# everpeace/kube-throttler

Measured on AMD Instinct MI355X. Metric: pod_throttle_decisions_per_sec, higher is better.
Workload: dtype int64; 1 GPU; configs[2]: 1M pods x 1k Throttle+ClusterThrottle, D=8; pods_total=1000000, pods_per_gpu=1000000, throttles=1000, dims=8, labels_per_pod=8, namespaces=64, step=reconcile(aggregate+allreduce+finalize,apply)+check(all pods), streams=one, kernel_variant=indexed, parallelism=pods row-sharded x1, throttles replicated, exchange=none

## Files before the change

### kube_throttler_amd/csrc/kt_kernels_check.hip

```cpp
#include <type_traits>

#include "kt_scan.h"

#ifdef KT_PROFILE_PHASES
__device__ unsigned long long kt_prof_check[16];
extern "C" int kt_debug_prof_check(unsigned long long* out16, int reset) {
  if (hipMemcpyFromSymbol(out16, HIP_SYMBOL(kt_prof_check), 16 * 8) != hipSuccess) return -1;
  if (reset) { unsigned long long z[16] = {0}; (void)hipMemcpyToSymbol(HIP_SYMBOL(kt_prof_check), z, 16 * 8); }
  return 0;
}
#define KT_PROF_T(var) const unsigned long long var = __builtin_amdgcn_s_memtime()
#define KT_PROF_ADD(slot, dt) prof_acc[slot] += (dt)
#else
#define KT_PROF_T(var)
#define KT_PROF_ADD(slot, dt)
#endif

namespace kt {


constexpr uint32_t kListCap = 128;
template <int DT>
struct alignas(16) WordVerdict {
  uint64_t seg_lo, seg_hi;
  uint64_t tight;
  uint64_t exc;
  uint64_t act;
  uint64_t ins;
  uint64_t act_nib[DT / 4][16];
};
constexpr uint32_t kTiAdj = 0x00100000u, kTiTight = 0x10000000u;
constexpr int kTiShActive = 16, kTiShIdle = 22;

template <int DT, bool WORDWISE, class TI, class WV>
__device__ __forceinline__ void build_term_verdicts(uint32_t tt, uint32_t c, const u32x2* g_rflags, TI* tinfo, WV* wv) {
  const bool real = (tt & kTermReal) != 0;
  const uint32_t t = tt & kTermRowMask;
  const u32x2 rf = real ? g_rflags[t] : u32x2{0u, 0u};
  u32x2 ti = {0u, 0u};
  if (real) {
    const uint32_t sh_act = (rf.x & kRecExceedsByCount) ? 4u : 24u;
    const uint32_t sh_idle = (rf.x & kRecExceedsByCount) ? 4u : (rf.x & kRecActiveByCount) ? 24u : (rf.x & kRecInsufficientByCount) ? 44u : 0u;
    ti.x = t | ((tt & kTermAdj) ? kTiAdj : 0u);
    ti.y = (rf.y & 0xFFFFu) | sh_act << kTiShActive | sh_idle << kTiShIdle | ((rf.x & kRecTight) ? kTiTight : 0u);
  }
  tinfo[c] = ti;
  if (WORDWISE) {
    const uint32_t ln = c & 63u;
    const uint32_t tp = (uint32_t)__shfl_up((int)tt, 1), tn = (uint32_t)__shfl_down((int)tt, 1);
    const bool adj = (tt & kTermAdj) != 0;
    const bool same_prev = ln > 0u && adj && (tp & kTermReal) && (tp & kTermAdj) && (tp & kTermRowMask) == t;
    const bool same_next = ln < 63u && adj && (tn & kTermReal) && (tn & kTermAdj) && (tn & kTermRowMask) == t;
    const bool xc = (rf.x & kRecExceedsByCount) != 0;
    const uint64_t m_lo = __ballot(real && !same_prev), m_hi = __ballot(real && !same_next);
    const uint64_t m_tight = __ballot(real && (rf.x & kRecTight) != 0), m_exc = __ballot(real && xc);
    const uint64_t m_act = __ballot(real && (rf.x & kRecActiveByCount) != 0), m_ins = __ballot(real && (rf.x & kRecInsufficientByCount) != 0);
    WV* wvp = wv + (c >> 6);
    const uint64_t mine = ln == 0u ? m_lo : ln == 1u ? m_hi : ln == 2u ? m_tight : ln == 3u ? m_exc : ln == 4u ? m_act : m_ins;
    const uint32_t eq = ln >> 4, ev = ln & 15u;
    uint64_t tab = m_act;
#pragma unroll
    for (int d = 0; d < DT; ++d) {
      const uint64_t m = __ballot(real && ((rf.y >> d) & 1u) != 0);
      tab |= ((uint32_t)(d >> 2) == eq && ((ev >> (d & 3)) & 1u)) ? m : 0ull;
    }
    typedef decltype(&wvp->seg_lo) u64p;
    if (ln < 6u) ((u64p)wvp)[ln] = mine;
    if (ln < 4u * (uint32_t)DT) ((u64p)wvp)[6u + ln] = tab;
  }
}
template <int DT>
__host__ __device__ constexpr uint32_t verdict_image_word_bytes() { return 64u * 8u; }

template <int DT>
__global__ __launch_bounds__(256) void kt_build_verdict_images(const unsigned char* blob, const BmChunk* chunks, const void* recs, int T,
                                                               uint32_t total_words, unsigned char* out) {
  const BmChunk ch = chunks[blockIdx.y];
  const uint32_t w = blockIdx.x * 4u + (threadIdx.x >> 6);
  if (w >= ch.n_words) return;
  const u32x2* g_rflags = (const u32x2*)rec_flags<DT>((void*)recs, T);
  const uint32_t* term_t = (const uint32_t*)(blob + ch.img_off + ch.off_term_t);
  const uint32_t c_local = w * 64u + (threadIdx.x & 63u);
  const uint32_t c_glob = (ch.w0 + w) * 64u + (threadIdx.x & 63u);
  build_term_verdicts<DT, true>(term_t[c_local], c_glob, g_rflags, (u32x2*)out, (WordVerdict<DT>*)(out + (size_t)total_words * 64u * 8u));
}
size_t verdict_images_bytes(uint32_t total_words, int D) {
  return (size_t)total_words * (64u * 8u + (D <= 8 ? sizeof(WordVerdict<8>) : sizeof(WordVerdict<16>))) + 64;
}
void launch_build_verdict_images(const IndexDev& ix, uint32_t total_words, const void* recs, int T, int D, void* out, hipStream_t s) {
  if (!ix.n_chunks || !ix.bm_max_words) return;
  const dim3 g_((ix.bm_max_words + 3u) / 4u, ix.n_chunks), b_(256);
  if (dt_bucket_ix(D) <= 8) hipLaunchKernelGGL(kt_build_verdict_images<8>, g_, b_, 0, s, ix.bm_blob, ix.bm_chunks, recs, T, total_words, (unsigned char*)out);
  else hipLaunchKernelGGL(kt_build_verdict_images<16>, g_, b_, 0, s, ix.bm_blob, ix.bm_chunks, recs, T, total_words, (unsigned char*)out);
}

template <bool CACHED>
struct TileMatchWords {};
template <>
struct TileMatchWords<true> {
  uint64_t mx[kMatchReplay];
};
template <int LA, int NV = 1, bool CACHED = false>
struct TileRec : TileMatchWords<CACHED> {
  uint32_t p;
  uint64_t meta;
  u32x4 raw[LA / 8];
  unsigned long long carried;
  int64_t v[NV];
};

struct BmCheckArgs {
  const uint64_t* meta;
  const uint16_t* latom;
  const int64_t* req;
  const uint32_t* lpair;
  const uint32_t* lkey;
  const int64_t* rows;
  const void* recs;
  uint64_t* summary;
  uint8_t* status;
  const SelProgram* sp;
  const uint8_t* ns_valid;
  const uint32_t* slow_thr;
  int64_t n;
  BmIndexArgs ix;
  uint32_t off_cnt, off_list, off_tinfo, off_wv;
  uint32_t off_next;
  uint32_t n_slow;
  int32_t DS, LS, T;
  uint32_t* ticket;
  uint64_t* host_summary;
  uint32_t has_overflow;
  const uint64_t* v_meta;
  const uint16_t* v_latom;
  uint64_t* carry;
  const uint32_t* wg_range;
  uint32_t n_inline;
  int64_t inline_rows[8];
  const unsigned char* wv_img;
  uint32_t wv_total_words;
  unsigned char* slab;
  uint32_t* slab_tag;
  uint32_t epoch;
  uint32_t off_rank, off_tab;
  uint32_t pk_nw, pk_rec;
  uint32_t pk_dim[8];
  MatchCacheArgs mc;
};

static BmCheckArgs make_bm_check_args(const PodTable& pods, int64_t n, const int64_t* rows, const SelProgram& sp,
                                      const SelProgram* sp_dev, const IndexDev& ix, const void* recs,
                                      uint64_t* summary, uint8_t* status, uint32_t* total, const PackPlan* agg_pk = nullptr) {
  BmCheckArgs a{};
  a.meta = pods.meta, a.latom = pods.latom, a.req = pods.req, a.lpair = pods.lpair, a.lkey = pods.lkey;
  a.n = n, a.rows = rows, a.recs = recs, a.summary = summary, a.status = status;
  a.sp = sp_dev, a.ns_valid = sp.ns_valid, a.slow_thr = ix.slow_thr, a.n_slow = ix.n_slow;
  a.DS = pods.DS, a.LS = pods.LS, a.T = sp.T;
  uint32_t o = 0;
  auto take = [&](uint32_t bytes) { uint32_t r = o; o += (bytes + 15u) & ~15u; return r; };
  a.off_cnt = take(kBlockIx * 8);
  a.off_list = take((kBlockIx / kWave) * kListCap * 4);
  a.off_next = take(16);
  a.off_tinfo = take(ix.bm_max_words * 64u * 8u);
  a.off_wv = take(ix.bm_max_words * (uint32_t)(pods.D <= 8 ? sizeof(WordVerdict<8>) : sizeof(WordVerdict<16>)));
  plan_bitmap_index(ix, a.ix, take);
  if (agg_pk) {
    a.pk_nw = agg_pk->nw, a.pk_rec = agg_pk->rec_bytes;
    for (int d = 0; d < 8; ++d)
      a.pk_dim[d] = (uint32_t)agg_pk->shift[d] | (uint32_t)agg_pk->pos[d] << 8 | (uint32_t)agg_pk->word[d] << 16 | (agg_pk->width[d] ? 1u << 24 : 0u);
    a.off_rank = take(ix.bm_max_words * 64u * 2u);
    a.off_tab = take(ix.bm_max_thr * agg_pk->rec_bytes);
  }
  *total = o;
  return a;
}

int check_sweep_blocks(int64_t n) {
  const int64_t nb = (n + kBlockIx - 1) / kBlockIx;
  return (int)(nb > kCUs ? kCUs : nb < 1 ? 1 : nb);
}
uint32_t check_fixed_lds() { return kBlockIx * 8 + (kBlockIx / kWave) * kListCap * 4 + 64; }
static_assert(sizeof(WordVerdict<16>) == 560 && 64u * 8u + sizeof(WordVerdict<16>) == kCheckWordLds, "kCheckWordLds (kt_index.h) follows WordVerdict");
static_assert(sizeof(WordVerdict<8>) == 304, "WordVerdict<8>");
uint32_t check_word_lds(int D) { return 64u * 8u + (uint32_t)(D <= 8 ? sizeof(WordVerdict<8>) : sizeof(WordVerdict<16>)); }

template <int DT, int LA, bool VETO, int NEED, int WPE, bool FULL, bool SMALL, bool ONE = false, bool AGG = false, bool CACHED = false>
__global__ __launch_bounds__(kBlockIx, WPE) void kt_check_bitmap(const BmCheckArgs a) {
  static_assert(!AGG || (ONE && !FULL && !SMALL && WPE < 8), "the fused sweep is the lean single-chunk form, one workgroup per CU");
  static_assert(!CACHED || (ONE && !FULL && !SMALL && !AGG && WPE >= 8 && !VETO && NEED == 2 && DT == 8), "the cached form is the lean two-per-CU sweep (one instantiation: nothing of the scan's form is left in it)");
  constexpr int kDrainUnroll = WPE >= 8 ? 1 : (DT / 2 > 4 ? 4 : DT / 2);
  constexpr int kDrainFinalUnroll = WPE >= 8 ? 2 : (DT / 2 > 4 ? 4 : DT / 2);
  constexpr bool WORDWISE = !FULL;
  constexpr bool PREFETCH = WPE < 8;
#ifdef KT_PROFILE_PHASES
  unsigned long long prof_acc[8] = {0, 0, 0, 0, 0, 0, 0, 0};
  KT_PROF_T(t_kernel0);
#endif
  KT_LDS unsigned char* lds = (KT_LDS unsigned char*)kt_smem;
  const CheckRec<DT>* recs = (const CheckRec<DT>*)a.recs;
  const u32x2* g_rflags = (const u32x2*)rec_flags<DT>((void*)a.recs, a.T);
  const uint32_t n = (uint32_t)a.n;
  const int DS = a.DS;
  const uint32_t lane = threadIdx.x & (kWave - 1);
  const uint32_t wave = __builtin_amdgcn_readfirstlane(threadIdx.x / kWave);
  lds_u64wp cnt = (lds_u64wp)(lds + a.off_cnt) + wave * kWave;
  lds_u32wp list = (lds_u32wp)(lds + a.off_list) + wave * kListCap;
  KT_LDS u32x2* tinfo = (KT_LDS u32x2*)(lds + a.off_tinfo);
  const uint32_t n_wtiles = (n + kWave - 1) / kWave;
  const uint32_t wstep = gridDim.x * (kBlockIx / kWave);
  const uint32_t n_chunks = ONE ? 1u : a.ix.n_chunks;
  const uint32_t c_lo = SMALL ? blockIdx.x : 0u, c_hi = SMALL ? blockIdx.x + 1u : n_chunks;
  const bool by_ns = !SMALL && !ONE && a.ix.by_ns != 0u;
  uint32_t t_lo = 0, t_hi = n_wtiles, ns_lo = 0, ns_hi = 0, first_ci = 0u, last_ci = n_chunks - 1u;
  uint32_t rec0 = 0, rec_end = n;
  if (by_ns) {
    if (a.wg_range) {
      rec0 = __builtin_amdgcn_readfirstlane(a.wg_range[blockIdx.x]), rec_end = __builtin_amdgcn_readfirstlane(a.wg_range[blockIdx.x + 1u]);
      if (rec0 >= rec_end) return;
      t_lo = 0u, t_hi = (rec_end - rec0 + kWave - 1u) / kWave;
    } else {
      const uint32_t tpb = (n_wtiles + gridDim.x - 1u) / gridDim.x;
      t_lo = min(blockIdx.x * tpb, n_wtiles), t_hi = min(t_lo + tpb, n_wtiles);
      if (t_lo >= t_hi) return;
    }
    ns_lo = (uint32_t)(a.v_meta[(uint64_t)rec0 + (uint64_t)t_lo * kWave] & kMetaNsMask);
    ns_hi = (uint32_t)(a.v_meta[min((uint64_t)rec0 + (uint64_t)t_hi * kWave, (uint64_t)rec_end) - 1u] & kMetaNsMask);
    ns_lo = __builtin_amdgcn_readfirstlane(ns_lo), ns_hi = __builtin_amdgcn_readfirstlane(max(ns_hi, ns_lo));
    relevant_chunk_span(a.ix, ns_lo, ns_hi, first_ci, last_ci);
    last_ci = max(last_ci, first_ci);
  }
  for (uint32_t ci = SMALL ? c_lo : first_ci; ci < (SMALL ? c_hi : last_ci + 1u); ++ci) {
    if (by_ns && ci != first_ci && !chunk_relevant(a.ix, ci, ns_lo, ns_hi)) continue;
    const bool first = ONE || ci == (SMALL ? 0u : first_ci), last = ONE || ci == last_ci;
    const BmChunk ch = a.ix.chunks[ci];
    const uint32_t wt0 = SMALL ? (wave == 0 ? blockIdx.y : n_wtiles) : by_ns ? t_lo + wave : blockIdx.x * (kBlockIx / kWave) + wave;
    const uint32_t wt_step = SMALL ? n_wtiles : by_ns ? (uint32_t)(kBlockIx / kWave) : wstep;
    auto fetch_tile = [&](uint32_t wt) {
      TileRec<LA, AGG ? DT : 1, CACHED> r;
      const uint32_t i = rec0 + wt * kWave + lane;
      const uint32_t ic = min(i, rec_end - 1u);
      r.p = CACHED ? ic : (SMALL && a.n_inline) ? (uint32_t)a.inline_rows[ic & 7u] : a.rows ? (uint32_t)a.rows[ic] : ic;
      r.meta = by_ns ? a.v_meta[ic] : a.meta[r.p];
      if constexpr (CACHED) load_match_words(a.mc, r.p, r.mx);
      else load_atoms<LA>(by_ns ? a.v_latom : a.latom, by_ns ? ic : r.p, r.raw);
      const unsigned long long* carry_w = by_ns ? (const unsigned long long*)a.carry + ic : (const unsigned long long*)a.summary + (by_ns ? r.p : i);
      r.carried = (!SMALL && !first && i < rec_end) ? __hip_atomic_load(carry_w, __ATOMIC_RELAXED, __HIP_MEMORY_SCOPE_AGENT) : 0ull;
      if constexpr (AGG) load_requests<DT>(a.req, DS, (int64_t)r.p, r.v);
      return r;
    };
    TileRec<LA, AGG ? DT : 1, CACHED> cur{};
    KT_PROF_T(t_b0);
    __syncthreads();
    KT_PROF_T(t_b1);
    KT_PROF_ADD(0, t_b1 - t_b0);
    const BmView bm = open_chunk<VETO>(lds, a.ix, ch);
    if (by_ns && threadIdx.x == 0) *(lds_u32wp)(lds + a.off_next) = t_lo;
    const bool from_images = !SMALL && !ONE && !FULL && a.wv_img != nullptr;
    const uint32_t* term_t = (const uint32_t*)(a.ix.blob + ch.img_off + ch.off_term_t);
    uint32_t tt_first = 0u;
    if (!from_images && threadIdx.x < ch.n_words * 64u) tt_first = term_t[threadIdx.x];
    {
      const u32x4* img0 = (const u32x4*)(a.ix.blob + ch.img_off);
      StageSeg segs[4] = {chunk_image_segment(a.ix, ch), StageSeg{0u, img0, 0u}, StageSeg{0u, img0, 0u}, StageSeg{0u, img0, 0u}};
      if constexpr (CACHED)
        segs[0] = StageSeg{a.ix.lds_img + ch.off_nsl_rng, (const u32x4*)(a.ix.blob + ch.img_off + ch.off_nsl_rng), (ch.lds_bytes - ch.off_nsl_rng) / 16u};
      if constexpr (AGG) segs[1] = StageSeg{a.off_rank, (const u32x4*)(a.ix.blob + ch.img_off + ch.off_term_rank), ch.n_words * 8u};
      if (from_images) {
        segs[2] = StageSeg{a.off_tinfo, (const u32x4*)(a.wv_img + (size_t)ch.w0 * verdict_image_word_bytes<DT>()), ch.n_words * (64u * 8u / 16u)};
        if (WORDWISE)
          segs[3] = StageSeg{a.off_wv, (const u32x4*)(a.wv_img + (size_t)a.wv_total_words * 64u * 8u + (size_t)ch.w0 * sizeof(WordVerdict<DT>)),
                             ch.n_words * (uint32_t)(sizeof(WordVerdict<DT>) / 16u)};
      }
      lds_stage_segments<4>(lds, segs);
    }
    if constexpr (AGG) {
      const uint32_t tab_bytes = (ch.n_thr * a.pk_rec + 15u) & ~15u;
      for (uint32_t i = threadIdx.x; i < tab_bytes / 4; i += kBlockIx) ((lds_u32wp)(lds + a.off_tab))[i] = 0u;
    }
    if (from_images) {
    } else {
      for (uint32_t c = threadIdx.x; c < ch.n_words * 64u; c += kBlockIx)
        build_term_verdicts<DT, WORDWISE>(c == threadIdx.x ? tt_first : term_t[c], c, g_rflags, tinfo, (KT_LDS WordVerdict<DT>*)(lds + a.off_wv));
    }
    KT_PROF_T(t_b2);
    __syncthreads();
    KT_PROF_T(t_b3);
    KT_PROF_ADD(1, t_b2 - t_b1);
    KT_PROF_ADD(2, t_b3 - t_b2);
    KT_PROF_ADD(6, 1ull);
    auto next_tile = [&](uint32_t prev) -> uint32_t {
      if (by_ns) {
        uint32_t t = 0u;
        if (lane == 0u) t = lds_add((lds_u32wp)(lds + a.off_next), 1u);
        return __builtin_amdgcn_readfirstlane(t);
      }
      return prev + wt_step;
    };
    uint32_t wt = by_ns ? next_tile(0u) : wt0;
    uint32_t wt_next = 0u;
    for (; wt < t_hi; wt = wt_next) {
      KT_PROF_T(t_f0);
      cur = fetch_tile(wt);
#ifdef KT_PROFILE_PHASES
      __builtin_amdgcn_s_waitcnt(0);
      KT_PROF_T(t_f1);
      KT_PROF_ADD(3, t_f1 - t_f0);
      KT_PROF_ADD(7, 1ull);
#endif
      const uint32_t i = rec0 + wt * kWave + lane;
      const bool in = i < rec_end;
      const uint32_t ic = min(i, rec_end - 1u);
      const uint32_t p = cur.p;
      const uint32_t si = by_ns ? p : i;
      const uint64_t meta = cur.meta;
      u32x4 raw[LA / 8];
#pragma unroll
      for (int q = 0; q < LA / 8; ++q) raw[q] = CACHED ? u32x4{0u, 0u, 0u, 0u} : cur.raw[q];
      unsigned long long* carry_w = by_ns ? (unsigned long long*)a.carry + ic : (unsigned long long*)a.summary + si;
      const unsigned long long carried = cur.carried;
      cnt[lane] = 0ull;
      unsigned long long my = carried & ~3ull;
      const bool on = in && ((meta >> kMetaStateShift) & kPodValid) != 0;
      const uint32_t ns = on ? (uint32_t)(meta & kMetaNsMask) : 0u;
      const uint32_t nz = (uint32_t)(meta >> kMetaNzShift);
      const uint32_t ns_ok_raw = a.ns_valid[ns];
      bool pod_err = (carried & 2ull) != 0;
      uint32_t ro[LA];
      if constexpr (!CACHED) atom_row_offsets<LA>(raw, ro);
      uint32_t n_list = 0;
      uint32_t last_t = 0xFFFFFFFFu;
      bool counted = false;
      uint32_t zero_keys = 0u;
      unsigned long long pw[4] = {0ull, 0ull, 0ull, 0ull};
      if constexpr (AGG) {
        const uint32_t st = (uint32_t)(meta >> kMetaStateShift) & 0xFu;
        counted = in && (st & (kPodValid | kPodSchedMatch | kPodScheduled | kPodFinished)) == (kPodValid | kPodSchedMatch | kPodScheduled);
        const uint32_t present = (uint32_t)(meta >> kMetaPresentShift) & 0xFFFFu;
        zero_keys = present & ~nz & 0xFFFFu;
        pw[0] = 1ull;
        static_assert(!AGG || DT == 8, "pk_dim holds eight dimensions");
#pragma unroll
        for (int d = 0; d < 8; ++d) {
          const uint32_t pd = a.pk_dim[d];
          const uint64_t f = (uint64_t)cur.v[d] >> (pd & 63u);
          const uint64_t piece = (pd >> 24) ? f << ((pd >> 8) & 63u) : 0ull;
          const uint32_t k = (pd >> 16) & 3u;
          pw[0] |= k == 0u ? piece : 0ull, pw[1] |= k == 1u ? piece : 0ull, pw[2] |= k == 2u ? piece : 0ull, pw[3] |= k == 3u ? piece : 0ull;
        }
      }

      auto drain = [&](auto unroll_tag) {
        constexpr int UNROLL = decltype(unroll_tag)::value;
        for (uint32_t base = 0; base < n_list; base += kWave) {
          const uint32_t j = base + lane;
          const bool vv = j < n_list;
          const uint32_t e = list[vv ? j : 0u];
          const uint32_t pl = e >> 20;
          u32x2 ti = {0u, 0u};
          if (WORDWISE) ti = tinfo[e & kTermRowMask];
          const uint32_t t = WORDWISE ? ti.x & kTermRowMask : e & kTermRowMask;
          const uint32_t prow = (uint32_t)__shfl((int)p, (int)pl);
          const uint32_t psi = FULL ? (uint32_t)__shfl((int)si, (int)pl) : 0u;
          const uint32_t pnz = (uint32_t)__shfl((int)nz, (int)pl);
          const CheckRec<DT>* rc = recs + t;
          const kt_i64x2* xr = (const kt_i64x2*)(a.req + (uint64_t)prow * (uint32_t)DS);
          u32x2 fa;
          if (WORDWISE) {
            const uint32_t sh_act = (ti.y >> kTiShActive) & 63u, sh_idle = (ti.y >> kTiShIdle) & 63u;
            fa.x = (sh_act == 4u ? kRecExceedsByCount : 0u) | (sh_idle == 24u ? kRecActiveByCount : 0u) | (sh_idle == 44u ? kRecInsufficientByCount : 0u);
            fa.y = ti.y & 0xFFFFu;
          } else {
            fa = g_rflags[t];
          }
          bool exc = false, ins = false;
#pragma unroll 1
          for (int q0 = 0; q0 < DT / 2; q0 += UNROLL) {
            kt_i64x2 x[UNROLL], th[UNROLL], hd[UNROLL];
#pragma unroll
            for (int u = 0; u < UNROLL; ++u) {
              const int q = q0 + u;
              x[u] = xr[2 * q < DS ? q : 0];
// ... 87 lines not shown
#pragma unroll
        for (int k = 0; k < DT / 4; ++k) r.nib[k] = *(KT_LDS const unsigned long long*)(q + (PREFETCH ? nib_off[k] : nib_offset(k)));
        return r;
      };
      KT_LDS const uint16_t* trank = (KT_LDS const uint16_t*)(lds + a.off_rank);
      KT_LDS unsigned char* tab = lds + a.off_tab;
      const uint32_t pk_rec = AGG ? a.pk_rec : 0u, pk_nw = AGG ? a.pk_nw : 0u;
      auto fold = [&](uint32_t w, uint64_t x) {
        uint64_t xf = counted ? x : 0ull;
        auto add = [&](bool has, uint32_t r) {
          if (has) {
            KT_LDS unsigned char* rp = tab + __umul24(r, pk_rec);
            lds_u64wp tv = (lds_u64wp)rp;
            lds_add64(tv, pw[0]);
            if (pk_nw > 1u) lds_add64(tv + 1, pw[1]);
            if (pk_nw > 2u) lds_add64(tv + 2, pw[2]);
            if (pk_nw > 3u) lds_add64(tv + 3, pw[3]);
            if (zero_keys) (void)__hip_atomic_fetch_or((lds_u32wp)(rp + pk_nw * 8u), zero_keys, __ATOMIC_RELAXED, __HIP_MEMORY_SCOPE_WORKGROUP);
          }
        };
        while (__ballot(xf != 0ull) != 0ull) {
          const bool h1 = xf != 0ull;
          const uint32_t c1 = h1 ? w * 64u + (uint32_t)__ffsll((unsigned long long)xf) - 1u : 0u;
          xf &= xf - 1ull;
          const bool h2 = xf != 0ull;
          const uint32_t c2 = h2 ? w * 64u + (uint32_t)__ffsll((unsigned long long)xf) - 1u : 0u;
          xf &= xf - 1ull;
          const uint32_t r1 = trank[c1] & 0x7FFFu, r2 = trank[c2] & 0x7FFFu;
          add(h1, r1);
          add(h2, r2);
        }
      };
      auto settle = [&](uint32_t w, uint64_t x, const VerdictRegs& q) -> uint64_t {
        if (seg_on) {
          const uint64_t v = x | q.seg.y;
          x = andn_64(x, v - q.seg.x);
        }
        if constexpr (AGG) fold(w, x);
        uint64_t act = q.nib[0];
#pragma unroll
        for (int k = 1; k < DT / 4; ++k) act |= q.nib[k];
        const uint64_t xe = and_not_and_64(x, q.te.x, q.te.y);
        const uint64_t xf = and_not_not_64(x, q.te.x, q.te.y);
        const uint64_t xa = xf & act, xi = and_not_and_64(xf, act, q.ai.y);
        n_exc = (uint32_t)__popc((uint32_t)xe) + ((uint32_t)__popc((uint32_t)(xe >> 32)) + n_exc);
        n_act = (uint32_t)__popc((uint32_t)xa) + ((uint32_t)__popc((uint32_t)(xa >> 32)) + n_act);
        n_ins = (uint32_t)__popc((uint32_t)xi) + ((uint32_t)__popc((uint32_t)(xi >> 32)) + n_ins);
        return x & q.te.x;
      };
      auto confirm_slow = [&](uint32_t c) {
        return term_match_mem(*a.sp, bm.term_g[c], a.lpair + (uint64_t)p * (uint32_t)a.LS, a.lkey + (uint64_t)p * (uint32_t)a.LS, a.LS);
      };
      auto peel_tight = [&](bool has, uint32_t c) { push(has, c); };
      if constexpr (CACHED) {
        auto settle_word = [&](uint32_t w, uint64_t x, int) -> uint64_t { return settle(w, x, fetch(w)); };
        replay_tile(bm, scan_on, ns, cur.mx, a.mc.planes, peel_tight, settle_word, ScanNoPrefetch());
      } else if constexpr (PREFETCH) {
        scan_tile<LA, VETO, NEED, VETO>(
            bm, scan_on, ns, ro, peel_tight, confirm_slow,
            [&](uint32_t w, uint64_t x, const VerdictRegs& q) -> uint64_t { return settle(w, x, q); },
            [&](uint32_t w) -> VerdictRegs { return fetch(w); });
      } else {
        scan_tile<LA, VETO, NEED, false>(
            bm, scan_on, ns, ro, peel_tight, confirm_slow,
            [&](uint32_t w, uint64_t x, int) -> uint64_t {
              if (__ballot(x != 0ull) == 0ull) return 0ull;
              return settle(w, x, fetch(w));
            });
      }
      my = (unsigned long long)n_exc << 4 | (unsigned long long)n_act << 24 | (unsigned long long)n_ins << 44;
      }
      wt_next = next_tile(wt);
#ifdef KT_PROFILE_PHASES
      KT_PROF_T(t_s1);
      KT_PROF_ADD(4, t_s1 - t_f1);
#endif
      if (n_list) drain(std::integral_constant<int, kDrainFinalUnroll>());
      pod_err |= on & (ns_ok_raw == 0u);
      if (SMALL) {
        if (in) {
          const unsigned long long c = my + cnt[lane];
          if (c) (void)__hip_atomic_fetch_add((unsigned long long*)a.summary + i, c, __ATOMIC_RELAXED, __HIP_MEMORY_SCOPE_AGENT);
          if (pod_err) (void)__hip_atomic_fetch_or((unsigned long long*)a.summary + i, 2ull, __ATOMIC_RELAXED, __HIP_MEMORY_SCOPE_AGENT);
        }
        __threadfence();
        uint32_t arrived = 0;
        if (lane == 0) arrived = __hip_atomic_fetch_add(a.ticket + wt, 1u, __ATOMIC_ACQ_REL, __HIP_MEMORY_SCOPE_AGENT);
        arrived = __builtin_amdgcn_readfirstlane(arrived);
        if (arrived + 1u == n_chunks) {
          if (in) {
            const unsigned long long w = __hip_atomic_load((unsigned long long*)a.summary + i, __ATOMIC_RELAXED, __HIP_MEMORY_SCOPE_AGENT);
            const unsigned long long c = w & ~3ull;
            const unsigned long long fin = !on ? 0ull : (w & 2ull) ? 2ull : (c | (c ? 1ull : 0ull));
            a.summary[i] = fin;
            if (a.host_summary) a.host_summary[i] = fin;
            if (FULL && a.status && on && (w & 2ull))
              for (int t = 0; t < a.T; ++t) a.status[(uint64_t)i * (uint32_t)a.T + t] = 255;
          }
          if (lane == 0) a.ticket[wt] = 0u;
        }
      } else if (in) {
        const unsigned long long c = my + cnt[lane];
        if (last) {
          a.summary[si] = !on ? 0ull : pod_err ? 2ull : (c | (c ? 1ull : 0ull));
          if (FULL && a.status && pod_err)
            for (int t = 0; t < a.T; ++t) a.status[(uint64_t)si * (uint32_t)a.T + t] = 255;
        } else {
          *carry_w = c | (pod_err ? 2ull : 0ull);
        }
      }
#ifdef KT_PROFILE_PHASES
      __builtin_amdgcn_s_waitcnt(0);
      KT_PROF_T(t_d1);
      KT_PROF_ADD(5, t_d1 - t_s1);
#endif
    }
    if constexpr (AGG) {
      __syncthreads();
      const uint32_t tab_bytes = (ch.n_thr * a.pk_rec + 15u) & ~15u;
      u32x4* dst = (u32x4*)(a.slab + (size_t)ch.slab_off * 16 + (size_t)blockIdx.x * tab_bytes);
      lds_u4p src = (lds_u4p)(lds + a.off_tab);
      for (uint32_t i = threadIdx.x; i < tab_bytes / 16; i += kBlockIx) dst[i] = src[i];
      if (threadIdx.x == 0) a.slab_tag[ci * kSlabTagStride + blockIdx.x] = a.epoch;
    }
  }
#ifdef KT_PROFILE_PHASES
  if (!SMALL && lane == 0) {
    KT_PROF_T(t_kernel1);
    for (int k = 0; k < 8; ++k) atomicAdd(&kt_prof_check[k], prof_acc[k]);
    atomicAdd(&kt_prof_check[8], t_kernel1 - t_kernel0);
    atomicAdd(&kt_prof_check[9], 1ull);
  }
#endif
}

#define KT_BM_LAUNCH(DT_, LA_, VETO_, NEED_, WPE_, FULL_, SMALL_, ONE_)                                         \
  {                                                                                                             \
    auto kfn = kt_check_bitmap<DT_, LA_, VETO_, NEED_, WPE_, FULL_, SMALL_, ONE_>;                              \
    (void)hipFuncSetAttribute((const void*)kfn, hipFuncAttributeMaxDynamicSharedMemorySize, (int)lds_bytes);    \
    hipLaunchKernelGGL(kfn, g_, b_, lds_bytes, s, bm_args);                                                     \
  }
#define KT_BM_LAUNCH_CACHED()                                                                                   \
  {                                                                                                             \
    auto kfn = kt_check_bitmap<8, 8, false, 2, 8, false, false, true, false, true>;                             \
    (void)hipFuncSetAttribute((const void*)kfn, hipFuncAttributeMaxDynamicSharedMemorySize, (int)lds_bytes);    \
    hipLaunchKernelGGL(kfn, g_, b_, lds_bytes, s, bm_args);                                                     \
  }
#define KT_BM_CASE(DT_, LA_, VETO_, NEED_)                                                   \
  {                                                                                          \
    if (small) KT_BM_LAUNCH(DT_, LA_, VETO_, NEED_, 4, true, true, false)                    \
    else if (full) KT_BM_LAUNCH(DT_, LA_, VETO_, NEED_, 4, true, false, false)               \
    else if (cached) KT_BM_LAUNCH_CACHED()                                                   \
    else if (two_per_cu) KT_BM_LAUNCH(DT_, LA_, VETO_, NEED_, 8, false, false, true)         \
    else KT_BM_LAUNCH(DT_, LA_, VETO_, NEED_, 4, false, false, false)                        \
  }

#define KT_BM_CASE5(DT_, LA_)                                                           \
  {                                                                                     \
    if (small) KT_BM_LAUNCH(DT_, LA_, true, 5, 4, true, true, false)                    \
    else if (full) KT_BM_LAUNCH(DT_, LA_, true, 5, 4, true, false, false)               \
    else KT_BM_LAUNCH(DT_, LA_, true, 5, 4, false, false, false)                        \
  }

const char* launch_check_indexed(const PodTable& pods, int64_t n, const int64_t* rows_dev, const SelProgram& sp,
                          const SelProgram* sp_dev, const IndexDev& ix, const void* recs, uint64_t* summary,
                          uint8_t* status, hipStream_t s, const CheckSmall* sm, bool overflow_pods, const CheckByNs* by_ns, bool one_per_cu,
                          const MatchCacheArgs* mc) {
  if (n <= 0) return "";
  const int DT = dt_bucket_ix(pods.D), LA = pods.LA;
  if (status) (void)hipMemsetAsync(status, 0, (size_t)n * (size_t)sp.T, s);
  uint32_t bm_total = 0;
  BmCheckArgs bm_args = make_bm_check_args(pods, n, rows_dev, sp, sp_dev, ix, recs, summary, status, &bm_total);
  if (bm_total > (uint32_t)kMaxLds) return nullptr;
  const size_t lds_bytes = bm_total;
  const bool small = sm != nullptr && n <= kCheckSmallMax;
  if (small) {
    (void)hipMemsetAsync(summary, 0, (size_t)n * 8, s);
    bm_args.ticket = sm->ticket, bm_args.host_summary = sm->host_summary;
    bm_args.n_inline = sm->n_inline;
    for (int k = 0; k < 8; ++k) bm_args.inline_rows[k] = sm->inline_rows[k];
  }
  bm_args.has_overflow = overflow_pods ? 1u : 0u;
  if (by_ns && !small && rows_dev) {
    bm_args.ix.by_ns = 1u;
    bm_args.v_meta = by_ns->v_meta, bm_args.v_latom = by_ns->v_latom, bm_args.carry = by_ns->carry;
    bm_args.wv_img = by_ns->wv_img, bm_args.wv_total_words = by_ns->wv_total_words;
    bm_args.wg_range = by_ns->wg_range_G == check_sweep_blocks(n) ? by_ns->wg_range : nullptr;
  }
  const bool full = status != nullptr || ix.n_slow != 0 || overflow_pods || ix.has_long;
  const bool need5 = ix.max_need > 3u;
  const bool one = ix.n_chunks == 1 && bm_args.ix.by_ns == 0u;
  const bool two_per_cu = one && !full && !small && !need5 && !one_per_cu && LA <= 8 && 2 * bm_total <= (uint32_t)kMaxLds;
  const bool cached = two_per_cu && DT <= 8 && mc != nullptr && mc->mw != nullptr && rows_dev == nullptr && mc->planes >= 1u &&
                      mc->planes <= (uint32_t)kMatchReplay && (uint64_t)n <= mc->stride && match_cache_fits(ix);
  if (cached) bm_args.mc = *mc, mc->used = true;
  int64_t nb = (n + kBlockIx - 1) / kBlockIx;
  const int64_t max_b = two_per_cu ? 2 * kCUs : kCUs;
  if (nb > max_b) nb = max_b;
  if (nb != check_sweep_blocks(n)) bm_args.wg_range = nullptr;
  dim3 g_((unsigned)nb), b_(kBlockIx);
  if (small) g_ = dim3(ix.n_chunks, (unsigned)((n + kWave - 1) / kWave));
  static const bool dbg_lds = getenv("KT_DEBUG_LDS") != nullptr;
  if (dbg_lds) fprintf(stderr, "kt_check_bitmap: lds=%u (%d per CU) chunks=%u LA=%d veto=%u need=%u\n", bm_total, two_per_cu ? 2 : 1, ix.n_chunks, LA, ix.has_veto, ix.max_need);
  const bool rich = ix.rich;
#ifdef KT_FAST_BUILD
  KT_BM_CASE(8, 8, false, 2)
#else
  if (!rich) { if (DT <= 8) KT_BM_CASE(8, 8, false, 2) else KT_BM_CASE(16, 8, false, 2) }
  else if (need5) {
    if (LA <= 8) { if (DT <= 8) KT_BM_CASE5(8, 8) else KT_BM_CASE5(16, 8) }
    else if (LA <= 16) { if (DT <= 8) KT_BM_CASE5(8, 16) else KT_BM_CASE5(16, 16) }
    else { if (DT <= 8) KT_BM_CASE5(8, 32) else KT_BM_CASE5(16, 32) }
  }
  else if (LA <= 8) { if (DT <= 8) KT_BM_CASE(8, 8, true, 3) else KT_BM_CASE(16, 8, true, 3) }
  else if (LA <= 16) { if (DT <= 8) KT_BM_CASE(8, 16, true, 3) else KT_BM_CASE(16, 16, true, 3) }
  else { if (DT <= 8) KT_BM_CASE(8, 32, true, 3) else KT_BM_CASE(16, 32, true, 3) }
#endif
  return small ? "kt_check_bitmap_small" : ix.n_chunks == 1 ? "kt_check_bitmap" : "kt_check_bitmap_chunked";
}

bool check_replays_match_cache(const PodTable& pods, const SelProgram& sp, const IndexDev& ix, uint32_t planes, bool overflow_pods, bool one_per_cu) {
  uint32_t bm_total = 0;
  (void)make_bm_check_args(pods, 1, nullptr, sp, nullptr, ix, nullptr, nullptr, nullptr, &bm_total);
  if (bm_total > (uint32_t)kMaxLds) return false;
  const bool full = ix.n_slow != 0 || overflow_pods || ix.has_long;
  const bool need5 = ix.max_need > 3u;
  const bool two_per_cu = ix.n_chunks == 1 && !full && !need5 && !one_per_cu && pods.LA <= 8 && 2 * bm_total <= (uint32_t)kMaxLds;
  return two_per_cu && dt_bucket_ix(pods.D) <= 8 && planes >= 1u && planes <= (uint32_t)kMatchReplay && match_cache_fits(ix);
}

#define KT_SWEEP_CASE(DT_, LA_, VETO_, NEED_)                                                                   \
  {                                                                                                             \
    auto kfn = kt_check_bitmap<DT_, LA_, VETO_, NEED_, 4, false, false, true, true>;                            \
    (void)hipFuncSetAttribute((const void*)kfn, hipFuncAttributeMaxDynamicSharedMemorySize, (int)lds_bytes);    \
    hipLaunchKernelGGL(kfn, g_, b_, lds_bytes, s, bm_args);                                                     \
  }
const char* launch_sweep_indexed(const PodTable& pods, int64_t n, const SelProgram& sp, const SelProgram* sp_dev, const IndexDev& ix,
                                 const void* recs, uint64_t* summary, const PackPlan& pk, void* slab, uint32_t* slab_tag, uint32_t epoch,
                                 int* launched_blocks, hipStream_t s) {
  if (n <= 0 || ix.n_chunks != 1 || ix.n_slow != 0 || ix.has_long || ix.max_need > 3u || pk.nw == 0) return nullptr;
  const int DT = dt_bucket_ix(pods.D), LA = pods.LA;
  if (DT != 8) return nullptr;
  uint32_t bm_total = 0;
  BmCheckArgs bm_args = make_bm_check_args(pods, n, nullptr, sp, sp_dev, ix, recs, summary, nullptr, &bm_total, &pk);
  if (bm_total > (uint32_t)kMaxLds) return nullptr;
  bm_args.slab = (unsigned char*)slab, bm_args.slab_tag = slab_tag, bm_args.epoch = epoch;
  const size_t lds_bytes = bm_total;
  const int64_t nb = aggregate_blocks(n);
// ... 11 lines not shown
```

### kube_throttler_amd/csrc/kt_scan.h

```cpp
#pragma once
#include "kt_index_device.h"


namespace kt {

struct BmIndexArgs {
  const unsigned char* blob;
  const BmChunk* chunks;
  uint32_t n_chunks, n_rows;
  uint32_t lds_img;
  const uint32_t* chunk_ns;
  uint32_t ns_words;
  uint32_t by_ns;
};

template <class Take>
static inline void plan_bitmap_index(const IndexDev& ix, BmIndexArgs& a, Take&& take) {
  a.blob = ix.bm_blob, a.chunks = ix.bm_chunks;
  a.n_chunks = ix.n_chunks, a.n_rows = ix.bm_rows;
  a.lds_img = take(ix.bm_max_lds);
  a.chunk_ns = ix.bm_chunk_ns, a.ns_words = ix.ns_words, a.by_ns = 0u;
}

__device__ __forceinline__ bool chunk_relevant(const BmIndexArgs& a, uint32_t ci, uint32_t ns_lo, uint32_t ns_hi) {
// ... 267 lines not shown
          xx = mux_64(any, two, h0.y);
          xx = mux_64(xx, three, h1.x);
        }
        xx = and_not_and_64(xx, vet, (uint64_t)e.z | (uint64_t)e.w << 32);
        xx = adv ? xx : 0ull;
        if (b.has_slow) {
          uint64_t sl = xx & h1.y;
          while (sl) {
            const uint32_t bit = (uint32_t)__ffsll((unsigned long long)sl) - 1u;
            sl &= sl - 1ull;
            if (!confirm(w * 64u + bit)) xx &= ~(1ull << bit);
          }
        }
      } else {
        uint64_t any = h0.x, par = 0;
#pragma unroll
        for (int g8 = 0; g8 < LA / 8; ++g8) {
          uint64_t r[8];
#pragma unroll
          for (int l = 0; l < 8; ++l) {
            r[l] = *(KT_LDS const unsigned long long*)(col + ro[8 * g8 + l]);
            if (VETO) vet |= *(KT_LDS const unsigned long long*)(colv + ro[8 * g8 + l]);
          }
          any = or3_64(or3_64(r[0], r[1], r[2]), or3_64(r[3], r[4], r[5]), or3_64(r[6], r[7], any));
          if (NEED >= 2) par = xor3_64(xor3_64(r[0], r[1], r[2]), xor3_64(r[3], r[4], r[5]), xor3_64(r[6], r[7], par));
        }
        xx = any;
        if (NEED >= 2) xx = and_nand_64(any, par, h0.y);
        uint64_t slow = 0;
        if (VETO) {
          const u64x2 h1 = *(KT_LDS const u64x2*)((KT_LDS const unsigned char*)(b.hdr + w) + 16);
          slow = h1.y;
        }
        if (VETO) xx = and_not_and_64(xx, vet, (uint64_t)e.z | (uint64_t)e.w << 32);
        else xx &= (uint64_t)e.z | (uint64_t)e.w << 32;
        xx = adv ? xx : 0ull;
        if (VETO && b.has_slow) {
          uint64_t sl = xx & slow;
          while (sl) {
            const uint32_t bit = (uint32_t)__ffsll((unsigned long long)sl) - 1u;
            sl &= sl - 1ull;
            if (!confirm(w * 64u + bit)) xx &= ~(1ull << bit);
          }
        }
      }
      x = post(w, xx, pf);
    } else {
      break;
    }
  }
}


__device__ __forceinline__ void load_match_words(const MatchCacheArgs& m, uint32_t p, uint64_t (&x)[kMatchReplay]) {
  const uint64_t* q = m.mw + p;
#pragma unroll
  for (int j = 0; j < kMatchReplay; ++j) {
    x[j] = 0ull;
    if ((uint32_t)j < m.planes) x[j] = q[(uint64_t)j * m.stride];
  }
}

template <class Match, class Post, class Pre>
__device__ __forceinline__ void replay_tile(const BmView& b, bool lane_on, uint32_t ns, const uint64_t (&mx)[kMatchReplay], uint32_t planes,
                                            Match&& match, Post&& post, Pre&& pre) {
  const u32x2 rng = b.nsl_rng[ns];
  const uint32_t len = lane_on ? min(rng.y - rng.x, planes) : 0u;
#pragma unroll
  for (int k_ = 0; k_ < kMatchReplay; ++k_) {
    const uint32_t k = (uint32_t)k_;
    if (k >= planes) break;
    const bool adv = k < len;
    uint64_t x = adv ? mx[k_] : 0ull;
    if (__ballot(x != 0ull) == 0ull) continue;
    const uint32_t w = b.nsl[adv ? rng.x + k : 0u].w;
    x = post(w, x, pre(w));
    while (__ballot(x != 0ull) != 0ull) {
      const bool has = x != 0ull;
      const uint32_t c = has ? w * 64u + (uint32_t)__ffsll((unsigned long long)x) - 1u : 0u;
      x &= x - 1ull;
      match(has, c);
    }
  }
}

}
```

Measured before the change: 22910 billion decisions/s.

## Split cached check into dedicated lean kernel specialized per plane count

Replaces the CACHED template branch of the general bitmap check kernel with a standalone kernel that carries only the state the cached sweep needs: the single chunk is passed by value, plane count is a template parameter, and carry, rows and atom handling are dropped. Match-word loads go through relaxed wavefront-scope atomic loads so they are issued early, and the drain computes verdicts inline with a simpler list entry encoding. The aim is lower register pressure and less control overhead in the hot sweep at two workgroups per CU. In exchange the code is duplicated, four more instantiations are added, and the fast-build path now rejects plane counts other than four.

```diff
diff --git a/kube_throttler_amd/csrc/kt_kernels_check.hip b/kube_throttler_amd/csrc/kt_kernels_check.hip
--- a/kube_throttler_amd/csrc/kt_kernels_check.hip
+++ b/kube_throttler_amd/csrc/kt_kernels_check.hip
@@ -1,3 +1,4 @@
+#include <cassert>
 #include <type_traits>
 
 #include "kt_scan.h"
@@ -94,14 +95,8 @@
   else hipLaunchKernelGGL(kt_build_verdict_images<16>, g_, b_, 0, s, ix.bm_blob, ix.bm_chunks, recs, T, total_words, (unsigned char*)out);
 }
 
-template <bool CACHED>
-struct TileMatchWords {};
-template <>
-struct TileMatchWords<true> {
-  uint64_t mx[kMatchReplay];
-};
-template <int LA, int NV = 1, bool CACHED = false>
-struct TileRec : TileMatchWords<CACHED> {
+template <int LA, int NV = 1>
+struct TileRec {
   uint32_t p;
   uint64_t meta;
   u32x4 raw[LA / 8];
@@ -145,7 +140,6 @@
   uint32_t off_rank, off_tab;
   uint32_t pk_nw, pk_rec;
   uint32_t pk_dim[8];
-  MatchCacheArgs mc;
 };
 
 static BmCheckArgs make_bm_check_args(const PodTable& pods, int64_t n, const int64_t* rows, const SelProgram& sp,
@@ -184,10 +178,9 @@
 static_assert(sizeof(WordVerdict<8>) == 304, "WordVerdict<8>");
 uint32_t check_word_lds(int D) { return 64u * 8u + (uint32_t)(D <= 8 ? sizeof(WordVerdict<8>) : sizeof(WordVerdict<16>)); }
 
-template <int DT, int LA, bool VETO, int NEED, int WPE, bool FULL, bool SMALL, bool ONE = false, bool AGG = false, bool CACHED = false>
+template <int DT, int LA, bool VETO, int NEED, int WPE, bool FULL, bool SMALL, bool ONE = false, bool AGG = false>
 __global__ __launch_bounds__(kBlockIx, WPE) void kt_check_bitmap(const BmCheckArgs a) {
   static_assert(!AGG || (ONE && !FULL && !SMALL && WPE < 8), "the fused sweep is the lean single-chunk form, one workgroup per CU");
-  static_assert(!CACHED || (ONE && !FULL && !SMALL && !AGG && WPE >= 8 && !VETO && NEED == 2 && DT == 8), "the cached form is the lean two-per-CU sweep (one instantiation: nothing of the scan's form is left in it)");
   constexpr int kDrainUnroll = WPE >= 8 ? 1 : (DT / 2 > 4 ? 4 : DT / 2);
   constexpr int kDrainFinalUnroll = WPE >= 8 ? 2 : (DT / 2 > 4 ? 4 : DT / 2);
   constexpr bool WORDWISE = !FULL;
@@ -236,19 +229,18 @@
     const uint32_t wt0 = SMALL ? (wave == 0 ? blockIdx.y : n_wtiles) : by_ns ? t_lo + wave : blockIdx.x * (kBlockIx / kWave) + wave;
     const uint32_t wt_step = SMALL ? n_wtiles : by_ns ? (uint32_t)(kBlockIx / kWave) : wstep;
     auto fetch_tile = [&](uint32_t wt) {
-      TileRec<LA, AGG ? DT : 1, CACHED> r;
+      TileRec<LA, AGG ? DT : 1> r;
       const uint32_t i = rec0 + wt * kWave + lane;
       const uint32_t ic = min(i, rec_end - 1u);
-      r.p = CACHED ? ic : (SMALL && a.n_inline) ? (uint32_t)a.inline_rows[ic & 7u] : a.rows ? (uint32_t)a.rows[ic] : ic;
+      r.p = (SMALL && a.n_inline) ? (uint32_t)a.inline_rows[ic & 7u] : a.rows ? (uint32_t)a.rows[ic] : ic;
       r.meta = by_ns ? a.v_meta[ic] : a.meta[r.p];
-      if constexpr (CACHED) load_match_words(a.mc, r.p, r.mx);
-      else load_atoms<LA>(by_ns ? a.v_latom : a.latom, by_ns ? ic : r.p, r.raw);
+      load_atoms<LA>(by_ns ? a.v_latom : a.latom, by_ns ? ic : r.p, r.raw);
       const unsigned long long* carry_w = by_ns ? (const unsigned long long*)a.carry + ic : (const unsigned long long*)a.summary + (by_ns ? r.p : i);
       r.carried = (!SMALL && !first && i < rec_end) ? __hip_atomic_load(carry_w, __ATOMIC_RELAXED, __HIP_MEMORY_SCOPE_AGENT) : 0ull;
       if constexpr (AGG) load_requests<DT>(a.req, DS, (int64_t)r.p, r.v);
       return r;
     };
-    TileRec<LA, AGG ? DT : 1, CACHED> cur{};
+    TileRec<LA, AGG ? DT : 1> cur{};
     KT_PROF_T(t_b0);
     __syncthreads();
     KT_PROF_T(t_b1);
@@ -262,8 +254,6 @@
     {
       const u32x4* img0 = (const u32x4*)(a.ix.blob + ch.img_off);
       StageSeg segs[4] = {chunk_image_segment(a.ix, ch), StageSeg{0u, img0, 0u}, StageSeg{0u, img0, 0u}, StageSeg{0u, img0, 0u}};
-      if constexpr (CACHED)
-        segs[0] = StageSeg{a.ix.lds_img + ch.off_nsl_rng, (const u32x4*)(a.ix.blob + ch.img_off + ch.off_nsl_rng), (ch.lds_bytes - ch.off_nsl_rng) / 16u};
       if constexpr (AGG) segs[1] = StageSeg{a.off_rank, (const u32x4*)(a.ix.blob + ch.img_off + ch.off_term_rank), ch.n_words * 8u};
       if (from_images) {
         segs[2] = StageSeg{a.off_tinfo, (const u32x4*)(a.wv_img + (size_t)ch.w0 * verdict_image_word_bytes<DT>()), ch.n_words * (64u * 8u / 16u)};
@@ -315,7 +305,7 @@
       const uint64_t meta = cur.meta;
       u32x4 raw[LA / 8];
 #pragma unroll
-      for (int q = 0; q < LA / 8; ++q) raw[q] = CACHED ? u32x4{0u, 0u, 0u, 0u} : cur.raw[q];
+      for (int q = 0; q < LA / 8; ++q) raw[q] = cur.raw[q];
       unsigned long long* carry_w = by_ns ? (unsigned long long*)a.carry + ic : (unsigned long long*)a.summary + si;
       const unsigned long long carried = cur.carried;
       cnt[lane] = 0ull;
@@ -326,7 +316,7 @@
       const uint32_t ns_ok_raw = a.ns_valid[ns];
       bool pod_err = (carried & 2ull) != 0;
       uint32_t ro[LA];
-      if constexpr (!CACHED) atom_row_offsets<LA>(raw, ro);
+      atom_row_offsets<LA>(raw, ro);
       uint32_t n_list = 0;
       uint32_t last_t = 0xFFFFFFFFu;
       bool counted = false;
@@ -520,10 +510,7 @@
         return term_match_mem(*a.sp, bm.term_g[c], a.lpair + (uint64_t)p * (uint32_t)a.LS, a.lkey + (uint64_t)p * (uint32_t)a.LS, a.LS);
       };
       auto peel_tight = [&](bool has, uint32_t c) { push(has, c); };
-      if constexpr (CACHED) {
-        auto settle_word = [&](uint32_t w, uint64_t x, int) -> uint64_t { return settle(w, x, fetch(w)); };
-        replay_tile(bm, scan_on, ns, cur.mx, a.mc.planes, peel_tight, settle_word, ScanNoPrefetch());
-      } else if constexpr (PREFETCH) {
+      if constexpr (PREFETCH) {
         scan_tile<LA, VETO, NEED, VETO>(
             bm, scan_on, ns, ro, peel_tight, confirm_slow,
             [&](uint32_t w, uint64_t x, const VerdictRegs& q) -> uint64_t { return settle(w, x, q); },
@@ -602,23 +589,227 @@
 #endif
 }
 
+struct BmCheckCachedArgs {
+  const uint64_t* meta;
+  const int64_t* req;
+  const void* recs;
+  uint64_t* summary;
+  const uint8_t* ns_valid;
+  const uint64_t* mw;
+  uint64_t mw_stride;
+  const unsigned char* blob;
+  BmChunk ch;
+  uint32_t n;
+  int32_t DS, T;
+  uint32_t lds_img, off_cnt, off_list, off_tinfo, off_wv;
+};
+static_assert(kTermRowMask == (1u << 20) - 1u && kWave == 64, "a list entry is lane << 20 | term number");
+
+static BmCheckCachedArgs make_check_cached_args(const IndexDev& ix, uint32_t* total) {
+  BmCheckCachedArgs a{};
+  uint32_t o = 0;
+  auto take = [&](uint32_t bytes) { uint32_t r = o; o += (bytes + 15u) & ~15u; return r; };
+  a.off_cnt = take(kBlockIx * 8u);
+  a.off_list = take((kBlockIx / kWave) * kListCap * 4);
+  a.off_tinfo = take(ix.bm_max_words * 64u * 8u);
+  a.off_wv = take(ix.bm_max_words * (uint32_t)sizeof(WordVerdict<8>));
+  a.lds_img = take(ix.bm_max_lds);
+  *total = o;
+  return a;
+}
+
+template <int PL>
+__global__ __launch_bounds__(kBlockIx, 8) void kt_check_bitmap_cached(const BmCheckCachedArgs a) {
+  static_assert(PL >= 1 && PL <= kMatchReplay, "one instantiation per plane count");
+  constexpr int DT = 8;
+  KT_LDS unsigned char* lds = (KT_LDS unsigned char*)kt_smem;
+  const CheckRec<DT>* recs = (const CheckRec<DT>*)a.recs;
+  const u32x2* g_rflags = (const u32x2*)rec_flags<DT>((void*)a.recs, a.T);
+  const uint32_t n = a.n;
+  const int DS = a.DS;
+  const uint32_t lane = threadIdx.x & (kWave - 1);
+  const uint32_t wave = __builtin_amdgcn_readfirstlane(threadIdx.x / kWave);
+  lds_u64wp cnt = (lds_u64wp)(lds + a.off_cnt) + wave * kWave;
+  lds_u32wp list = (lds_u32wp)(lds + a.off_list) + wave * kListCap;
+  KT_LDS u32x2* tinfo = (KT_LDS u32x2*)(lds + a.off_tinfo);
+  KT_LDS const unsigned char* wv = lds + a.off_wv;
+  const BmChunk& ch = a.ch;
+  const uint32_t n_wtiles = (n + kWave - 1) / kWave;
+  const uint32_t wstep = gridDim.x * (kBlockIx / kWave);
+  BmIndexArgs ixa{};
+  ixa.blob = a.blob, ixa.lds_img = a.lds_img;
+  const BmView bm = open_chunk<false>(lds, ixa, ch);
+  {
+    const uint32_t* term_t = (const uint32_t*)(a.blob + ch.img_off + ch.off_term_t);
+    uint32_t tt_first = 0u;
+    if (threadIdx.x < ch.n_words * 64u) tt_first = term_t[threadIdx.x];
+    const StageSeg segs[1] = {StageSeg{a.lds_img + ch.off_nsl_rng, (const u32x4*)(a.blob + ch.img_off + ch.off_nsl_rng), (ch.lds_bytes - ch.off_nsl_rng) / 16u}};
+    lds_stage_segments<1>(lds, segs);
+    for (uint32_t c = threadIdx.x; c < ch.n_words * 64u; c += kBlockIx)
+      build_term_verdicts<DT, true>(c == threadIdx.x ? tt_first : term_t[c], c, g_rflags, tinfo, (KT_LDS WordVerdict<DT>*)(lds + a.off_wv));
+  }
+  __syncthreads();
+  const bool seg_on = ch.has_adj != 0u;
+
+  struct Rec {
+    uint64_t meta;
+    uint64_t mx[kMatchReplay];
+  };
+  auto fetch_tile = [&](uint32_t wt) {
+    Rec r{};
+    const uint32_t ic = min(wt * kWave + lane, n - 1u);
+    r.meta = ld_issued(a.meta + ic);
+    const uint64_t* q = a.mw + ic;
+#pragma unroll
+    for (int j = 0; j < PL; ++j) r.mx[j] = ld_issued(q + (uint64_t)j * a.mw_stride);
+    return r;
+  };
+  for (uint32_t wt = blockIdx.x * (kBlockIx / kWave) + wave; wt < n_wtiles; wt += wstep) {
+    const Rec r = fetch_tile(wt);
+    cnt[lane] = 0ull;
+    uint32_t n_list = 0;
+
+    auto drain = [&](auto unroll_tag) {
+      constexpr int UNROLL = decltype(unroll_tag)::value;
+      for (uint32_t base = 0; base < n_list; base += kWave) {
+        const uint32_t j = base + lane;
+        const bool vv = j < n_list;
+        const uint32_t e = list[vv ? j : 0u];
+        const uint32_t pl = e >> 20;
+        const u32x2 ti = tinfo[e & kTermRowMask];
+        const uint32_t t = ti.x & kTermRowMask;
+        const uint32_t prow = min(wt * kWave + pl, n - 1u);
+        static_assert(kMetaNzShift == 48, "the non-zero mask is the meta word's top 16 bits");
+        const uint32_t pnz = ((const uint16_t*)(a.meta + prow))[3];
+        const CheckRec<DT>* rc = recs + t;
+        const kt_i64x2* xr = (const kt_i64x2*)(a.req + (uint64_t)prow * (uint32_t)DS);
+        const uint32_t sh_act = (ti.y >> kTiShActive) & 63u, sh_idle = (ti.y >> kTiShIdle) & 63u;
+        const uint32_t fx = (sh_act == 4u ? kRecExceedsByCount : 0u) | (sh_idle == 24u ? kRecActiveByCount : 0u) | (sh_idle == 44u ? kRecInsufficientByCount : 0u);
+        const uint32_t fy = ti.y & 0xFFFFu;
+        bool exc = false, ins = false;
+        if constexpr (UNROLL == 0) {
+#pragma unroll 1
+          for (int d = 0; d < DT; ++d) {
+            const int64_t x = a.req[(uint64_t)prow * (uint32_t)DS + (uint32_t)(d < DS ? d : 0)], th = rc->thr[d], hd = rc->head[d];
+            const bool nzd = (pnz >> d) & 1u;
+            exc |= nzd && x > th, ins |= nzd && x > hd;
+          }
+        } else {
+#pragma unroll 1
+        for (int q0 = 0; q0 < DT / 2; q0 += UNROLL) {
+          kt_i64x2 x[UNROLL], th[UNROLL], hd[UNROLL];
+#pragma unroll
+          for (int u = 0; u < UNROLL; ++u) {
+            const int q = q0 + u;
+            x[u] = xr[2 * q < DS ? q : 0];
+            th[u] = *(const kt_i64x2*)(rc->thr + 2 * q);
+            hd[u] = *(const kt_i64x2*)(rc->head + 2 * q);
+          }
+#pragma unroll
+          for (int u = 0; u < UNROLL; ++u) {
+            const int q = q0 + u;
+            const bool nz0 = (pnz >> (2 * q)) & 1u, nz1 = (pnz >> (2 * q + 1)) & 1u;
+            exc |= (nz0 && x[u].x > th[u].x) || (nz1 && x[u].y > th[u].y);
+            ins |= (nz0 && x[u].x > hd[u].x) || (nz1 && x[u].y > hd[u].y);
+          }
+        }
+        }
+        exc |= (fx & kRecExceedsByCount) != 0, ins |= (fx & kRecInsufficientByCount) != 0;
+        const bool act = (fx & kRecActiveByCount) || (pnz & fy);
+        const uint32_t st = exc ? 4u : act ? 2u : ins ? 3u : 1u;
+        if (vv && st != 1u) lds_add64(cnt + pl, st == 4u ? 1ull << 4 : st == 2u ? 1ull << 24 : 1ull << 44);
+      }
+      n_list = 0;
+    };
+    auto push = [&](bool want, uint32_t e) {
+      const uint64_t mk = __ballot(want);
+      if (mk == 0ull) return;
+      if (want) list[n_list + lane_rank(mk)] = e;
+      n_list += (uint32_t)__popcll(mk);
+      if (n_list > kListCap - kWave) drain(std::integral_constant<int, 0>());
+    };
+    {
+      const uint64_t meta = r.meta;
+      const bool on = wt * kWave + lane < n && ((meta >> kMetaStateShift) & kPodValid) != 0;
+      const uint32_t ns = on ? (uint32_t)(meta & kMetaNsMask) : 0u;
+      const uint32_t nz = (uint32_t)(meta >> kMetaNzShift) & 0xFFFFu;
+      const uint32_t ns_ok_raw = a.ns_valid[ns];
+      auto nib_offset = [&](int q) { return (uint32_t)offsetof(WordVerdict<DT>, act_nib) + (uint32_t)q * 128u + ((nz >> (4 * q)) & 15u) * 8u; };
+      uint32_t n_exc = 0u, n_act = 0u, n_ins = 0u;
+      auto settle_word = [&](uint32_t w, uint64_t x, int) -> uint64_t {
+        KT_LDS const unsigned char* q = wv + __umul24(w, (uint32_t)sizeof(WordVerdict<DT>));
+        if (seg_on) {
+          const u64x2 seg = *(KT_LDS const u64x2*)(q + offsetof(WordVerdict<DT>, seg_lo));
+          const uint64_t v = x | seg.y;
+          x = andn_64(x, v - seg.x);
+        }
+        const u64x2 te = *(KT_LDS const u64x2*)(q + offsetof(WordVerdict<DT>, tight));
+        const u64x2 ai = *(KT_LDS const u64x2*)(q + offsetof(WordVerdict<DT>, act));
+        uint64_t act = *(KT_LDS const unsigned long long*)(q + nib_offset(0));
+#pragma unroll
+        for (int k = 1; k < DT / 4; ++k) act |= *(KT_LDS const unsigned long long*)(q + nib_offset(k));
+        const uint64_t xe = and_not_and_64(x, te.x, te.y);
+        const uint64_t xf = and_not_not_64(x, te.x, te.y);
+        const uint64_t xa = xf & act, xi = and_not_and_64(xf, act, ai.y);
+        n_exc = (uint32_t)__popc((uint32_t)xe) + ((uint32_t)__popc((uint32_t)(xe >> 32)) + n_exc);
+        n_act = (uint32_t)__popc((uint32_t)xa) + ((uint32_t)__popc((uint32_t)(xa >> 32)) + n_act);
+        n_ins = (uint32_t)__popc((uint32_t)xi) + ((uint32_t)__popc((uint32_t)(xi >> 32)) + n_ins);
+        return x & te.x;
+      };
+      replay_tile(bm, on, ns, r.mx, (uint32_t)PL, [&](bool has, uint32_t c) { push(has, lane << 20 | c); }, settle_word, ScanNoPrefetch());
+      const unsigned long long my = (unsigned long long)n_exc << 4 | (unsigned long long)n_act << 24 | (unsigned long long)n_ins << 44;
+      cnt[lane] += my | (on ? 1ull : 0ull) | ((on && ns_ok_raw == 0u) ? 2ull : 0ull);
+    }
+    if (n_list) drain(std::integral_constant<int, 2>());
+    if (wt * kWave + lane < n) {
+      const unsigned long long w = cnt[lane], c = w & ~3ull;
+      a.summary[wt * kWave + lane] = !(w & 1ull) ? 0ull : (w & 2ull) ? 2ull : (c | (c ? 1ull : 0ull));
+    }
+  }
+}
+
+static void launch_check_cached(const PodTable& pods, int64_t n, const SelProgram& sp, const IndexDev& ix, const void* recs, uint64_t* summary,
+                                const MatchCacheArgs& mc, dim3 grid, hipStream_t s) {
+  uint32_t total = 0;
+  BmCheckCachedArgs a = make_check_cached_args(ix, &total);
+  assert(2u * total <= (uint32_t)kMaxLds && (uint64_t)ix.bm_max_words * 64u <= (uint64_t)kTermRowMask + 1u);
+  a.meta = pods.meta, a.req = pods.req, a.recs = recs, a.summary = summary, a.ns_valid = sp.ns_valid;
+  a.mw = mc.mw, a.mw_stride = mc.stride;
+  a.blob = ix.bm_blob, a.ch = ix.h_chunks[0];
+  a.n = (uint32_t)n, a.DS = pods.DS, a.T = sp.T;
+  static const bool dbg_lds = getenv("KT_DEBUG_LDS") != nullptr;
+  if (dbg_lds) fprintf(stderr, "kt_check_bitmap_cached: lds=%u (2 per CU) workgroups=%u planes=%u\n", total, grid.x, mc.planes);
+#define KT_CHECK_CACHED_LAUNCH(PL_)                                                                             \
+  {                                                                                                             \
+    auto kfn = kt_check_bitmap_cached<PL_>;                                                                     \
+    (void)hipFuncSetAttribute((const void*)kfn, hipFuncAttributeMaxDynamicSharedMemorySize, (int)total);        \
+    hipLaunchKernelGGL(kfn, grid, dim3(kBlockIx), total, s, a);                                                 \
+  }
+  static_assert(kMatchReplay == 4, "one instantiation per plane count");
+#ifdef KT_FAST_BUILD
+  KT_CHECK_CACHED_LAUNCH(kMatchReplay)
+#else
+  switch (mc.planes) {
+    case 1: KT_CHECK_CACHED_LAUNCH(1) break;
+    case 2: KT_CHECK_CACHED_LAUNCH(2) break;
+    case 3: KT_CHECK_CACHED_LAUNCH(3) break;
+    default: KT_CHECK_CACHED_LAUNCH(4) break;
+  }
+#endif
+#undef KT_CHECK_CACHED_LAUNCH
+}
+
 #define KT_BM_LAUNCH(DT_, LA_, VETO_, NEED_, WPE_, FULL_, SMALL_, ONE_)                                         \
   {                                                                                                             \
     auto kfn = kt_check_bitmap<DT_, LA_, VETO_, NEED_, WPE_, FULL_, SMALL_, ONE_>;                              \
     (void)hipFuncSetAttribute((const void*)kfn, hipFuncAttributeMaxDynamicSharedMemorySize, (int)lds_bytes);    \
     hipLaunchKernelGGL(kfn, g_, b_, lds_bytes, s, bm_args);                                                     \
   }
-#define KT_BM_LAUNCH_CACHED()                                                                                   \
-  {                                                                                                             \
-    auto kfn = kt_check_bitmap<8, 8, false, 2, 8, false, false, true, false, true>;                             \
-    (void)hipFuncSetAttribute((const void*)kfn, hipFuncAttributeMaxDynamicSharedMemorySize, (int)lds_bytes);    \
-    hipLaunchKernelGGL(kfn, g_, b_, lds_bytes, s, bm_args);                                                     \
-  }
 #define KT_BM_CASE(DT_, LA_, VETO_, NEED_)                                                   \
   {                                                                                          \
     if (small) KT_BM_LAUNCH(DT_, LA_, VETO_, NEED_, 4, true, true, false)                    \
     else if (full) KT_BM_LAUNCH(DT_, LA_, VETO_, NEED_, 4, true, false, false)               \
-    else if (cached) KT_BM_LAUNCH_CACHED()                                                   \
+    else if (cached) launch_check_cached(pods, n, sp, ix, recs, summary, *mc, g_, s); \
     else if (two_per_cu) KT_BM_LAUNCH(DT_, LA_, VETO_, NEED_, 8, false, false, true)         \
     else KT_BM_LAUNCH(DT_, LA_, VETO_, NEED_, 4, false, false, false)                        \
   }
@@ -661,7 +852,10 @@
   const bool two_per_cu = one && !full && !small && !need5 && !one_per_cu && LA <= 8 && 2 * bm_total <= (uint32_t)kMaxLds;
   const bool cached = two_per_cu && DT <= 8 && mc != nullptr && mc->mw != nullptr && rows_dev == nullptr && mc->planes >= 1u &&
                       mc->planes <= (uint32_t)kMatchReplay && (uint64_t)n <= mc->stride && match_cache_fits(ix);
-  if (cached) bm_args.mc = *mc, mc->used = true;
+#ifdef KT_FAST_BUILD
+  if (cached && mc->planes != (uint32_t)kMatchReplay) return nullptr;
+#endif
+  if (cached) mc->used = true;
   int64_t nb = (n + kBlockIx - 1) / kBlockIx;
   const int64_t max_b = two_per_cu ? 2 * kCUs : kCUs;
   if (nb > max_b) nb = max_b;
diff --git a/kube_throttler_amd/csrc/kt_scan.h b/kube_throttler_amd/csrc/kt_scan.h
--- a/kube_throttler_amd/csrc/kt_scan.h
+++ b/kube_throttler_amd/csrc/kt_scan.h
@@ -343,13 +343,8 @@
 }
 
 
-__device__ __forceinline__ void load_match_words(const MatchCacheArgs& m, uint32_t p, uint64_t (&x)[kMatchReplay]) {
-  const uint64_t* q = m.mw + p;
-#pragma unroll
-  for (int j = 0; j < kMatchReplay; ++j) {
-    x[j] = 0ull;
-    if ((uint32_t)j < m.planes) x[j] = q[(uint64_t)j * m.stride];
-  }
+__device__ __forceinline__ uint64_t ld_issued(const uint64_t* p) {
+  return __hip_atomic_load(p, __ATOMIC_RELAXED, __HIP_MEMORY_SCOPE_WAVEFRONT);
 }
 
 template <class Match, class Post, class Pre>
```

Result: faster. 23650 billion decisions/s (median of 6 runs) (+3.2%).
